# akamiru/bce

Measured on AMD Instinct MI355X. Metric: MB/s compressed, higher is better.
Workload: dtype u8/u32 integer

## Files before the change

bce_amd/csrc/common.h:

```cpp
#pragma once
#include <hip/hip_runtime.h>
#include <stdint.h>
#include <stdio.h>
#include <stdlib.h>
#include <string.h>

#include <atomic>
#include <chrono>
#include <condition_variable>
#include <exception>
#include <new>
#include <memory>
#include <mutex>
#include <thread>
#include <vector>

#include <sys/mman.h>

#include "../../include/bce_hip.h"
#include "bce_core.h"
#include "host_coder.h"

namespace bce {

// ... 194 lines not shown
    hipError_t _e = (expr);                                           \
    if (_e != hipSuccess) return bce::set_err((ctx), _e, #expr, __LINE__); \
  } while (0)

#define BCE_TRY(expr)                 \
  do {                                \
    int _rc = (expr);                 \
    if (_rc != BCE_HIP_OK) return _rc; \
  } while (0)

size_t ctx_trim(bce_hip_ctx *c);
inline bool test_oom_now() {
  static const char *e = getenv("BCE_HIP_TEST_OOM");
  static const unsigned long k = e ? strtoul(e, nullptr, 10) : 0;
  static std::atomic<unsigned long> count{0};
  return k && (count.fetch_add(1) + 1) % k == 0;
}
enum AllocSite { kAllocPlain = 0, kAllocListFirst = 1, kAllocListFallback = 2 };
inline bool test_oom_fails(const bce_hip_ctx *c, int site, int attempt) {
  switch (c->dbg_oom) {
    case 1: return site == kAllocListFirst;
    case 2: return site != kAllocPlain;
    case 3: return attempt == 0;
    default: return false;
  }
}
inline size_t test_oom_bytes(size_t bytes) {
  size_t fr = 0, tot = 0;
  if (hipMemGetInfo(&fr, &tot) != hipSuccess) { (void)hipGetLastError(); return bytes; }
  return tot + ((size_t)1 << 30);
}
inline int ensure(bce_hip_ctx *c, DevBuf &b, size_t bytes, int site = kAllocPlain) {
  if (bytes <= b.cap) return BCE_HIP_OK;
  if (b.p) {
    for (hipStream_t st : {c->stream, c->k4_stream, c->copy_stream}) if (st) BCE_HIP_TRY(c, hipStreamSynchronize(st));
    (void)hipFree(b.p);
    b.p = nullptr; b.cap = 0;
  }
  const double t0 = now_s();
  const bool hooked = c->dbg_oom != 0;
  hipError_t e = hipMalloc(&b.p, test_oom_fails(c, site, 0) ? test_oom_bytes(bytes) : bytes);
  const bool pretend = e == hipSuccess && test_oom_now();
  if (pretend) { (void)hipFree(b.p); e = hipErrorOutOfMemory; }
  if (e == hipErrorOutOfMemory) {
    (void)hipGetLastError();
    b.p = nullptr;
    if (ctx_trim(c) || pretend || hooked) e = hipMalloc(&b.p, test_oom_fails(c, site, 1) ? test_oom_bytes(bytes) : bytes);
  }
  if (e != hipSuccess) {
    b.p = nullptr;
    if (e == hipErrorOutOfMemory) (void)hipGetLastError();
    BCE_HIP_TRY(c, e);
  }
  c->alloc_s += now_s() - t0; c->alloc_bytes += bytes; c->alloc_calls++;
  if (now_s() - t0 > 0.02 && getenv("BCE_ALLOC_TRACE")) fprintf(stderr, "alloc: hipMalloc of %.1f MB took %.3f s\n", bytes / 1e6, now_s() - t0);
  b.cap = bytes;
  return BCE_HIP_OK;
}
inline int pin_alloc(bce_hip_ctx *c, void **p, size_t bytes) {
  const double t0 = now_s();
  BCE_HIP_TRY(c, hipHostMalloc(p, bytes, hipHostMallocDefault));
  c->pin_s += now_s() - t0; c->pin_bytes += bytes; c->pin_calls++;
  return BCE_HIP_OK;
}
inline void release(DevBuf &b) {
  if (b.p) (void)hipFree(b.p);
  b.p = nullptr; b.cap = 0;
}

inline int read_back(bce_hip_ctx *c, void *dst, const void *dev_src, size_t bytes) {
  if (bytes > 4096) return BCE_HIP_E_ARG;
  if (!c->h_small) BCE_TRY(pin_alloc(c, &c->h_small, 4096));
  BCE_HIP_TRY(c, hipMemcpyAsync(c->h_small, dev_src, bytes, hipMemcpyDeviceToHost, c->stream));
  BCE_HIP_TRY(c, hipStreamSynchronize(c->stream));
  memcpy(dst, c->h_small, bytes);
  return BCE_HIP_OK;
}

template <class F>
inline int bce_guarded(bce_hip_ctx *c, F &&body) {
  try { return body(); }
  catch (const std::bad_alloc &) { if (c) snprintf(c->err, sizeof c->err, "host allocation failed"); return BCE_HIP_E_NOMEM; }
  catch (const std::exception &e) { if (c) snprintf(c->err, sizeof c->err, "%s", e.what()); return BCE_HIP_E_INTERNAL; }
  catch (...) { if (c) snprintf(c->err, sizeof c->err, "unknown exception"); return BCE_HIP_E_INTERNAL; }
}

struct PhaseScope {
  PhaseScope(bce_hip_ctx *c, int phase) : c_(c) { c_->phase = phase; }
  ~PhaseScope() { c_->phase = 0; }
  PhaseScope(const PhaseScope &) = delete;
  PhaseScope &operator=(const PhaseScope &) = delete;
 private:
  bce_hip_ctx *c_;
};

struct RoctxRange {
  explicit RoctxRange(const char *name);
  ~RoctxRange();
  RoctxRange(const RoctxRange &) = delete;
  RoctxRange &operator=(const RoctxRange &) = delete;
 private:
  bool on_;
};

constexpr uint32_t K3_TAIL_CAP = 1024;
constexpr uint32_t K3_SMALL_MAXTILES = 2048;
#ifndef K3_SMALL_NODES_VALUE
#define K3_SMALL_NODES_VALUE 2000000u
#endif
constexpr uint32_t K3_SMALL_NODES = K3_SMALL_NODES_VALUE;
constexpr uint32_t K3_TAIL_ENTER = 512;
constexpr uint32_t K3_TAIL_MAXROUNDS = 65536;

inline uint32_t ceil_log2(uint32_t v) { uint32_t b = 0; while ((1ull << b) < v) ++b; return b; }

int k1_bwt(bce_hip_ctx *c);
int k1_divbwt(bce_hip_ctx *c, const uint8_t *T_host, uint8_t *U_host, uint32_t n, uint32_t *pidx);
int kd_inverse_bw_transform(bce_hip_ctx *c, const uint8_t *T_host, uint8_t *U_host, uint32_t n, uint32_t idx);
int kd_compare(bce_hip_ctx *c, const uint8_t *a, const uint8_t *b, uint64_t m, uint64_t *first_diff);
int kd_crc32(bce_hip_ctx *c, const uint8_t *d, uint64_t n, uint32_t *crc);
int k2_build_planes(bce_hip_ctx *c);
int k2_get_plane_bits(bce_hip_ctx *c, int plane, uint8_t *out);
int k2_rank1(bce_hip_ctx *c, int plane, const uint32_t *idx, uint32_t count, uint32_t *out);
int k3_begin(bce_hip_ctx *c);
int k3_rounds(bce_hip_ctx *c, uint32_t count, uint64_t nodes_hint);
int k3_rounds_small(bce_hip_ctx *c, uint32_t count, uint64_t cur_nodes, bool growing);
int k3_round_masked(bce_hip_ctx *c, uint32_t mask, bool repeat);
int k3_clear_need_flush(bce_hip_ctx *c);
int k3_clear_small_bail(bce_hip_ctx *c);
int k3_dfs_tail(bce_hip_ctx *c, const EnumCtl &ctl, uint32_t enter, bool *done);
int k3_tail(bce_hip_ctx *c, uint32_t max_rounds = K3_TAIL_MAXROUNDS);
int k3_fetch_tail_runs(bce_hip_ctx *c, uint32_t rounds);
int k3_sync_ctl(bce_hip_ctx *c, EnumCtl *out);
int k3_fetch_runs(bce_hip_ctx *c, uint32_t first_round, uint32_t count);
int k3_get_nodes(bce_hip_ctx *c, int plane, uint32_t *out, uint32_t cap, uint32_t *count);
int k3_reset_symbols(bce_hip_ctx *c);
int k3_grow_symbols(bce_hip_ctx *c, uint64_t cap);
int k4_prepare(bce_hip_ctx *c);
int k3_grow_lists(bce_hip_ctx *c, const EnumCtl &ctl);
uint64_t k3_symbol_capacity(const bce_hip_ctx *c, uint32_t n);
void k4_prepin(bce_hip_ctx *c, uint32_t n);
void k4_prepin_join(bce_hip_ctx *c, bool drop);
int k4_flush(bce_hip_ctx *c, uint64_t nsym, FlushSlot &slot);
int k4_flush_async(bce_hip_ctx *c, uint64_t nsym, FlushSlot &slot, bool copy_out = true);
int k4_long_runs(bce_hip_ctx *c, uint64_t nsym, uint32_t *count);
int k4_cost_begin(bce_hip_ctx *c);
int k4_cost_async(bce_hip_ctx *c, uint64_t nsym, FlushSlot &slot);
int k4_cost_end(bce_hip_ctx *c, uint64_t acc[16]);

int radix_sort_pairs(bce_hip_ctx *c, uint32_t *key[2], uint32_t *val[2], uint32_t n, uint32_t first_bit, uint32_t bits, int *res,
                     uint32_t max_digit_bits = 8);
int radix_sort_pairs_on(bce_hip_ctx *c, hipStream_t stream, DevBuf &hist, uint32_t *key[2], uint32_t *val[2], uint32_t n,
                        uint32_t first_bit, uint32_t bits, int *res, uint32_t max_digit_bits = 8);
int radix_sort_wide(bce_hip_ctx *c, uint32_t *lo[2], uint32_t *hi[2], uint32_t *val[2], uint32_t n, uint32_t bits, int *res,
                    uint32_t max_digit_bits = 10);
bool k4_in_flight(bce_hip_ctx *c);

}
```

bce_amd/csrc/k1_bwt.hip:

```cpp
#include <stdlib.h>

#include <utility>

#include "common.h"
#include "scan_util.h"

namespace bce {

#ifndef K1_ACT_TENTHS
#define K1_ACT_TENTHS 6
#endif

constexpr int K1_T = 256;

constexpr uint32_t K1_MAXB = 1024;
struct K1Plan { uint32_t nb, per_block; };
static K1Plan k1_plan(uint32_t n) {
  const uint32_t chunk = 2048;
  uint32_t chunks = (uint32_t)(((uint64_t)n + chunk - 1) / chunk);
  if (!chunks) chunks = 1;
  uint32_t nb = chunks < K1_MAXB ? chunks : K1_MAXB;
  uint32_t cpb = (chunks + nb - 1) / nb;
  nb = (chunks + cpb - 1) / cpb;
  return {nb, cpb * chunk};
// ... 569 lines not shown
  for (uint64_t i = (uint64_t)blockIdx.x * K1_T + threadIdx.x; i < m; i += (uint64_t)gridDim.x * K1_T)
    if (!(flag[i] & KF_DEFER)) rank[vs[i]] = nr[i];
}

template <int PASS, int MODE>
__global__ __launch_bounds__(K1_T) void k1_relist_kernel(const uint32_t *__restrict__ A, const uint32_t *__restrict__ vs,
                                                         const uint8_t *__restrict__ flag, uint32_t m,
                                                         uint32_t per_block, uint32_t nb, uint32_t *__restrict__ blockcnt,
                                                         uint32_t *__restrict__ out, uint32_t *__restrict__ out2, uint32_t *__restrict__ total,
                                                         uint32_t *__restrict__ blockcnt2 = nullptr, uint32_t *__restrict__ out3 = nullptr) {
  const uint64_t beg = (uint64_t)blockIdx.x * per_block;
  uint64_t end = beg + per_block;
  if (end > m) end = m;
  auto take = [&](uint64_t i) -> bool { return MODE == 0 ? (flag[i] & KF_DEFER) != 0 : (flag[i] & KF_KEEP) != 0; };
  if (PASS == 0) {
    uint32_t cnt = 0, hc = 0;
    for (uint64_t i = beg + threadIdx.x; i < end; i += K1_T) {
      const bool k = take(i);
      cnt += k ? 1u : 0u;
      if (MODE == 0) hc += (k && (A[i] & K1_HEAD)) ? 1u : 0u;
    }
    cnt = block_reduce_sum<K1_T>(cnt);
    if (MODE == 0) hc = block_reduce_sum<K1_T>(hc);
    if (threadIdx.x == 0) { blockcnt[blockIdx.x] = cnt; if (MODE == 0) blockcnt2[blockIdx.x] = hc; }
  } else {
    uint32_t b = 0, a = 0, b2 = 0, a2 = 0;
    for (uint32_t k = threadIdx.x; k < nb; k += K1_T) {
      const uint32_t v = blockcnt[k];
      a += v; if (k < blockIdx.x) b += v;
      if (MODE == 0) { const uint32_t v2 = blockcnt2[k]; a2 += v2; if (k < blockIdx.x) b2 += v2; }
    }
    uint32_t base = block_reduce_sum<K1_T>(b);
    const uint32_t all = block_reduce_sum<K1_T>(a);
    uint32_t hbase = 0;
    if (MODE == 0) {
      hbase = block_reduce_sum<K1_T>(b2);
      const uint32_t all2 = block_reduce_sum<K1_T>(a2);
      if (blockIdx.x == 0 && threadIdx.x == 0) total[1] = all2;
    }
    if (blockIdx.x == 0 && threadIdx.x == 0) total[0] = all;
    for (uint64_t c0 = beg; c0 < end; c0 += K1_T) {
      const uint64_t i = c0 + threadIdx.x;
      const bool k = i < end && take(i);
      const uint32_t a_i = (MODE == 0 && k) ? A[i] : 0u;
      uint32_t tot;
      const uint32_t ex = block_excl_scan_sum<K1_T>(k ? 1u : 0u, &tot);
      uint32_t htot = 0, hex = 0;
      const uint32_t hd = (MODE == 0 && (a_i & K1_HEAD)) ? 1u : 0u;
      if (MODE == 0) hex = block_excl_scan_sum<K1_T>(hd, &htot);
      if (k) {
        if (MODE == 0) { out[base + ex] = (uint32_t)i; out2[base + ex] = a_i & K1_SLOT; out3[base + ex] = hbase + hex + hd - 1u; }
        else { out[base + ex] = (A[i] & K1_SLOT) | ((flag[i] & KF_HEAD) ? K1_HEAD : 0u); out2[base + ex] = vs[i]; }
      }
      base += tot;
      hbase += htot;
    }
  }
}

__global__ __launch_bounds__(K1_T) void k1_big_gather_kernel(const uint32_t *__restrict__ idx, const uint32_t *__restrict__ gid,
                                                             const uint32_t *__restrict__ V, const uint32_t *__restrict__ rank,
                                                             uint32_t n, uint32_t nd, uint32_t h, uint32_t rbits,
                                                             uint32_t *__restrict__ lo, uint32_t *__restrict__ hi, uint32_t *__restrict__ val) {
  for (uint64_t j = (uint64_t)blockIdx.x * K1_T + threadIdx.x; j < nd; j += (uint64_t)gridDim.x * K1_T) {
    const uint32_t p = V[idx[j]];
    uint64_t q = (uint64_t)p + h;
    if (q >= n) q -= n;
    const uint64_t key = ((uint64_t)gid[j] << rbits) | rank[q];
    lo[j] = (uint32_t)key;
    hi[j] = (uint32_t)(key >> 32);
    val[j] = p;
  }
}
__global__ __launch_bounds__(K1_T) void k1_big_heads_kernel(const uint32_t *__restrict__ slots, const uint32_t *__restrict__ lo,
                                                            const uint32_t *__restrict__ hi, const uint32_t *__restrict__ val,
                                                            uint32_t nd, uint32_t per_block, uint32_t *__restrict__ sa,
                                                            uint32_t *__restrict__ nrk, uint32_t *__restrict__ blockmax) {
  const uint64_t beg = (uint64_t)blockIdx.x * per_block;
  uint64_t end = beg + per_block;
  if (end > nd) end = nd;
  uint32_t mx = 0;
  for (uint64_t j = beg + threadIdx.x; j < end; j += K1_T) {
    const uint32_t slot = slots[j];
    sa[slot] = val[j];
    const bool head = j == 0 || lo[j] != lo[j - 1] || hi[j] != hi[j - 1];
    nrk[j] = head ? slot : 0u;
    if (head) mx = slot;
  }
  mx = block_reduce_max<K1_T>(mx);
  if (threadIdx.x == 0) blockmax[blockIdx.x] = mx;
}

__global__ __launch_bounds__(K1_T) void k1_defer_flags_kernel(const uint32_t *__restrict__ nrk, const uint32_t *__restrict__ idx,
                                                              const uint32_t *__restrict__ sorted, uint32_t nd,
                                                              uint8_t *__restrict__ flag, uint32_t *__restrict__ vs) {
  for (uint64_t j = (uint64_t)blockIdx.x * K1_T + threadIdx.x; j < nd; j += (uint64_t)gridDim.x * K1_T) {
    const bool hd = j == 0 || nrk[j] != 0u;
    const bool nx = j + 1 >= nd || nrk[j + 1] != 0u;
    const uint32_t i = idx[j];
    flag[i] = (uint8_t)(KF_DEFER | (hd ? KF_HEAD : 0) | ((hd && nx) ? 0 : KF_KEEP));
    vs[i] = sorted[j];
  }
}

static int k1_sort_rotations(bce_hip_ctx *c, const uint8_t *T, uint32_t n, bool sentinel) {
  if (getenv("BCE_K1_V1")) return k1_sort_rotations_v1(c, T, n, sentinel);
  const size_t b4 = (size_t)n * 4;
  for (int i = 0; i < 2; ++i) { BCE_TRY(ensure(c, c->sa[i], b4)); BCE_TRY(ensure(c, c->key[i], b4)); BCE_TRY(ensure(c, c->khi[i], b4)); }
  BCE_TRY(ensure(c, c->rank, b4));
  BCE_TRY(ensure(c, c->k2, b4));
  BCE_TRY(ensure(c, c->nrk, b4));
  BCE_TRY(ensure(c, c->kflag, (size_t)n + 16));
  for (int i = 0; i < 2; ++i) { BCE_TRY(ensure(c, c->act[i], b4)); BCE_TRY(ensure(c, c->actv[i], b4)); }
  const K1Plan pl = k1_plan(n);
  BCE_TRY(ensure(c, c->blk, (size_t)(K1_MAXB + K1_SC_CODE + 128 + K1_MAXB) * 4));
  uint32_t *blockmax = c->blk.as<uint32_t>();
  uint32_t *scalars = blockmax + K1_MAXB;
  uint32_t *rank = c->rank.as<uint32_t>(), *k2 = c->k2.as<uint32_t>(), *nrk = c->nrk.as<uint32_t>();
  uint8_t *flag = c->kflag.as<uint8_t>();
  const uint32_t g = grid_for(n);
  const bool trace = getenv("BCE_K1_TRACE") != nullptr;
  double t_prev = now_s();
  auto lap = [&](const char *what, uint64_t h, uint32_t m, uint32_t nd) {
    if (!trace) return;
    (void)hipStreamSynchronize(c->stream);
    const double t = now_s();
    fprintf(stderr, "k1 %p: %-10s h %llu active %u deferred %u (+%.2f ms)\n", (void *)c, what, (unsigned long long)h, m, nd, (t - t_prev) * 1e3);
    t_prev = t;
  };

  const uint32_t nbytes = sentinel ? n - 1u : n;
  BCE_HIP_TRY(c, hipMemsetAsync(scalars + K1_SC_HIST, 0, 256 * 4, c->stream));
  hipLaunchKernelGGL(k1_bytehist_kernel, dim3(g < 1024u ? g : 1024u), dim3(K1_T), 0, c->stream, T, nbytes, scalars + K1_SC_HIST);
  uint32_t hist[256];
  BCE_TRY(read_back(c, hist, scalars + K1_SC_HIST, sizeof hist));
  uint16_t code[256];
  uint32_t sigma = sentinel ? 1u : 0u;
  for (int b = 0; b < 256; ++b) { code[b] = (uint16_t)sigma; if (hist[b]) ++sigma; }
  uint32_t bits = ceil_log2(sigma);
  if (bits < 1) bits = 1;
  uint32_t nsym = 64u / bits;
  if (nsym > 16u) nsym = 16u;
  if (const char *e = getenv("BCE_K1_KEYBITS")) { const uint32_t v = (uint32_t)strtoul(e, nullptr, 10); if (v >= bits && v / bits < nsym) nsym = v / bits; }
  const uint32_t keybits = nsym * bits;
  {
    if (!c->h_small) BCE_TRY(pin_alloc(c, &c->h_small, 4096));
    memcpy(c->h_small, code, sizeof code);
    BCE_HIP_TRY(c, hipMemcpyAsync(scalars + K1_SC_CODE, c->h_small, sizeof code, hipMemcpyHostToDevice, c->stream));
  }

  uint32_t *lo[2] = {c->key[0].as<uint32_t>(), c->key[1].as<uint32_t>()};
  uint32_t *hi[2] = {c->khi[0].as<uint32_t>(), c->khi[1].as<uint32_t>()};
  uint32_t *val[2] = {c->sa[0].as<uint32_t>(), c->sa[1].as<uint32_t>()};
  {
    const uint32_t per = K1_T * K1I_E;
    hipLaunchKernelGGL(k1_init64_kernel, dim3((uint32_t)(((uint64_t)n + per - 1) / per)), dim3(K1_T), 0, c->stream, T, n, nbytes,
                       reinterpret_cast<const uint16_t *>(scalars + K1_SC_CODE), bits, nsym, lo[0], hi[0], val[0]);
  }
  int res = 0;
  BCE_TRY(radix_sort_wide(c, lo, hi, val, n, keybits, &res, 9));
  lap("first sort", nsym, n, 0);
  BCE_HIP_TRY(c, hipMemsetAsync(scalars, 0, 16, c->stream));
  hipLaunchKernelGGL(k1_heads_kernel, dim3(pl.nb), dim3(K1_T), 0, c->stream, hi[res], lo[res], n, pl.per_block, nrk, blockmax, scalars);
  const uint32_t rbits = ceil_log2(n);
  static const uint32_t part_min = getenv("BCE_K1_PART_MIN") ? (uint32_t)strtoul(getenv("BCE_K1_PART_MIN"), nullptr, 10) : K1_PART_MIN;
  const bool sorted_apply = n >= part_min;
  if (sorted_apply) hipLaunchKernelGGL(k1_headidx_kernel, dim3(pl.nb), dim3(K1_T), 0, c->stream, nrk, blockmax, n, pl.per_block, k2);
  else hipLaunchKernelGGL(k1_apply_kernel, dim3(pl.nb), dim3(K1_T), 0, c->stream, nrk, blockmax, n, pl.per_block, val[res], rank);
  uint32_t *act[2] = {c->act[0].as<uint32_t>(), c->act[1].as<uint32_t>()};
  uint32_t *actv[2] = {c->actv[0].as<uint32_t>(), c->actv[1].as<uint32_t>()};
  uint32_t m = 0;
  hipLaunchKernelGGL(k1_active_kernel<0>, dim3(pl.nb), dim3(K1_T), 0, c->stream, nrk, (const uint32_t *)nullptr, n, pl.per_block, pl.nb,
                     blockmax, act[0], scalars + 2, 1u, (const uint32_t *)val[res], actv[0]);
  hipLaunchKernelGGL(k1_active_kernel<1>, dim3(pl.nb), dim3(K1_T), 0, c->stream, nrk, (const uint32_t *)nullptr, n, pl.per_block, pl.nb,
                     blockmax, act[0], scalars + 2, 1u, (const uint32_t *)val[res], actv[0]);
  if (sorted_apply) {
    const uint32_t b1 = rbits / ((rbits + 9u) / 10u);
    uint32_t *pk[2] = {val[res], lo[res ^ 1]}, *pv[2] = {k2, rank};
    int pr = 0;
    BCE_TRY(radix_sort_pairs(c, pk, pv, n, 0, b1, &pr, 10));
    uint32_t *qk[2] = {lo[res ^ 1], hi[res ^ 1]}, *qv[2] = {rank, val[res ^ 1]};
    BCE_TRY(radix_sort_pairs(c, qk, qv, n, b1, rbits - b1, &pr, 10));
    if (pr) BCE_HIP_TRY(c, hipMemcpyAsync(rank, qv[1], (size_t)n * 4, hipMemcpyDeviceToDevice, c->stream));
  }
  BCE_TRY(read_back(c, &m, scalars + 2, 4));
  lap("first ranks", nsym, m, 0);

  uint64_t h = nsym;
  uint32_t *sa = val[res];
  uint32_t *nr = hi[0], *vs = hi[1];
  while (m > 0 && h < n) {
    const uint32_t *A = act[0];
    const uint32_t nblk = (uint32_t)(((uint64_t)m + SEG_CH - 1) / SEG_CH);
    BCE_HIP_TRY(c, hipMemsetAsync(scalars + 3, 0, 4, c->stream));
    hipLaunchKernelGGL(k1_seg_sort_kernel, dim3(nblk), dim3(SEG_T), 0, c->stream, A, (const uint32_t *)actv[0], m, sa, rank, n, (uint32_t)h, nr, vs,
                       flag, scalars + 3);
    uint32_t nd = 0;
    BCE_TRY(read_back(c, &nd, scalars + 3, 4));
    const K1Plan ap = k1_plan(m);
    if (nd) {
      BCE_TRY(ensure(c, c->dl[0], (size_t)nd * 4));
      BCE_TRY(ensure(c, c->dl[1], (size_t)nd * 4));
      BCE_TRY(ensure(c, c->dl[2], (size_t)nd * 4));
      BCE_TRY(ensure(c, c->dl[3], (size_t)nd * 4));
      uint32_t *idx = c->dl[0].as<uint32_t>(), *slots = c->dl[1].as<uint32_t>(), *gid = c->dl[2].as<uint32_t>();
      uint32_t *blockcnt2 = scalars + K1_SC_CODE + 128;
      hipLaunchKernelGGL((k1_relist_kernel<0, 0>), dim3(ap.nb), dim3(K1_T), 0, c->stream, A, (const uint32_t *)vs, flag, m, ap.per_block, ap.nb, blockmax, idx, slots,
                         scalars + 4, blockcnt2, gid);
      hipLaunchKernelGGL((k1_relist_kernel<1, 0>), dim3(ap.nb), dim3(K1_T), 0, c->stream, A, (const uint32_t *)vs, flag, m, ap.per_block, ap.nb, blockmax, idx, slots,
                         scalars + 4, blockcnt2, gid);
      uint32_t cnts[2] = {0, 0};
      BCE_TRY(read_back(c, cnts, scalars + 4, 8));
      if (cnts[0] != nd || cnts[1] == 0 || cnts[1] > nd) { snprintf(c->err, sizeof c->err, "k1: deferred list %u / %u groups, expected %u elements", cnts[0], cnts[1], nd); return BCE_HIP_E_INTERNAL; }
      const uint32_t gbits = ceil_log2(cnts[1]);
      uint32_t *bl[2] = {lo[0], lo[1]};
      uint32_t *bh[2] = {val[res ^ 1], k2};
      uint32_t *bv[2] = {nrk, c->dl[3].as<uint32_t>()};
      const uint32_t ga = grid_for(nd);
      hipLaunchKernelGGL(k1_big_gather_kernel, dim3(ga), dim3(K1_T), 0, c->stream, idx, gid, (const uint32_t *)actv[0], rank, n, nd, (uint32_t)h, rbits,
                         bl[0], bh[0], bv[0]);
      int rb = 0;
      BCE_TRY(radix_sort_wide(c, bl, bh, bv, nd, rbits + gbits, &rb, 9));
      const K1Plan dp = k1_plan(nd);
      uint32_t *snrk = bv[rb ^ 1];
      hipLaunchKernelGGL(k1_big_heads_kernel, dim3(dp.nb), dim3(K1_T), 0, c->stream, slots, bl[rb], bh[rb], bv[rb], nd, dp.per_block, sa, snrk, blockmax);
      hipLaunchKernelGGL(k1_act_apply_kernel, dim3(dp.nb), dim3(K1_T), 0, c->stream, snrk, blockmax, nd, dp.per_block, bv[rb], rank);
      uint32_t *vjr = bv[rb];
      hipLaunchKernelGGL(k1_defer_flags_kernel, dim3(ga), dim3(K1_T), 0, c->stream, snrk, idx, (const uint32_t *)vjr, nd, flag, vs);
    }
    if (m >= part_min) {
      const uint32_t b1 = rbits / ((rbits + 9u) / 10u);
      uint32_t *pk[2] = {lo[0], lo[1]}, *pv[2] = {nr, k2};
      hipLaunchKernelGGL(k1_seg_pairs_kernel, dim3(grid_for(m)), dim3(K1_T), 0, c->stream, (const uint32_t *)vs, (const uint8_t *)flag, KF_DEFER, m, pk[0]);
      int pr = 0;
      BCE_TRY(radix_sort_pairs(c, pk, pv, m, 0, b1, &pr, 10));
      uint32_t *qk[2] = {lo[1], lo[0]}, *qv[2] = {k2, val[res ^ 1]};
      BCE_TRY(radix_sort_pairs(c, qk, qv, m, b1, rbits - b1, &pr, 10));
      hipLaunchKernelGGL(k1_scatter32_kernel, dim3(grid_for(m)), dim3(K1_T), 0, c->stream, (const uint32_t *)qk[pr], (const uint32_t *)qv[pr], m, n, rank);
    } else {
      hipLaunchKernelGGL(k1_seg_apply_kernel, dim3(grid_for(m)), dim3(K1_T), 0, c->stream, nr, vs, flag, m, rank);
    }
    hipLaunchKernelGGL((k1_relist_kernel<0, 1>), dim3(ap.nb), dim3(K1_T), 0, c->stream, A, (const uint32_t *)vs, flag, m, ap.per_block, ap.nb, blockmax, act[1],
                       actv[1], scalars + 2);
    hipLaunchKernelGGL((k1_relist_kernel<1, 1>), dim3(ap.nb), dim3(K1_T), 0, c->stream, A, (const uint32_t *)vs, flag, m, ap.per_block, ap.nb, blockmax, act[1],
                       actv[1], scalars + 2);
    const uint32_t m_old = m;
    BCE_TRY(read_back(c, &m, scalars + 2, 4));
    std::swap(act[0], act[1]);
    std::swap(actv[0], actv[1]);
    h <<= 1;
    c->stats.sort_rounds++;
    lap("round", h, m, nd);
    (void)m_old;
  }
  BCE_HIP_TRY(c, hipGetLastError());
  c->k1_unique = m == 0;
  c->sa_res = res;
  return BCE_HIP_OK;
}

int k1_bwt(bce_hip_ctx *c) {
  const uint32_t n = c->n;
  uint8_t *T = c->text.as<uint8_t>();
  BCE_TRY(ensure(c, c->bwt, n));
  uint8_t *bwt = c->bwt.as<uint8_t>();
  c->stats.sort_rounds = 0;
  c->k1_unique = false;
  c->k1_valid = false;
  if (n == 1) {
    BCE_HIP_TRY(c, hipMemcpyAsync(bwt, T, 1, hipMemcpyDeviceToDevice, c->stream));
    BCE_HIP_TRY(c, hipStreamSynchronize(c->stream));
    c->offset = 0;
    return BCE_HIP_OK;
  }
  BCE_TRY(k1_sort_rotations(c, T, n, false));
  const uint32_t g = grid_for(n);
  uint32_t *scalars = c->blk.as<uint32_t>() + K1_MAXB;
  const uint32_t *sa = c->sa[c->sa_res].as<uint32_t>();
  BCE_HIP_TRY(c, hipMemsetAsync(scalars + 1, 0xFF, 4, c->stream));
  hipLaunchKernelGGL(k1_bwt_kernel, dim3(g), dim3(K1_T), 0, c->stream, T, sa, n, bwt);
  hipLaunchKernelGGL(k1_offset_kernel, dim3(g), dim3(K1_T), 0, c->stream, c->rank.as<uint32_t>(), n, scalars + 1);
  uint32_t off = 0;
  BCE_TRY(read_back(c, &off, scalars + 1, 4));
  BCE_HIP_TRY(c, hipGetLastError());
  if (off >= n) { snprintf(c->err, sizeof c->err, "k1: no rank-0 rotation found"); return BCE_HIP_E_INTERNAL; }
  c->offset = off;
  c->k1_valid = true;
  return BCE_HIP_OK;
}

__global__ __launch_bounds__(K1_T) void k1_divbwt_gather_kernel(const uint8_t *__restrict__ T, const uint32_t *__restrict__ sa,
                                                                uint32_t m, uint32_t pidx, uint8_t *__restrict__ U) {
  for (uint64_t j = (uint64_t)blockIdx.x * K1_T + threadIdx.x; j < m; j += (uint64_t)gridDim.x * K1_T) {
    const uint32_t p = sa[j];
    if (p != 0u) U[j < pidx ? j : j - 1u] = T[p - 1u];
  }
}

int k1_divbwt(bce_hip_ctx *c, const uint8_t *T_host, uint8_t *U_host, uint32_t n, uint32_t *pidx_out) {
  if (n == 0 || n >= 0x7FFFFFFFu) return BCE_HIP_E_ARG;
  const uint32_t m = n + 1u;
  c->stage = 0; c->k1_valid = false; c->enum_active = false; c->text_loaded = false;
  BCE_TRY(ensure(c, c->text, m));
  BCE_TRY(ensure(c, c->bwt, m));
  uint8_t *T = c->text.as<uint8_t>();
  BCE_HIP_TRY(c, hipMemcpyAsync(T, T_host, n, hipMemcpyHostToDevice, c->stream));
  c->stats.sort_rounds = 0;
  BCE_TRY(k1_sort_rotations(c, T, m, true));
  uint32_t pidx = 0;
  BCE_TRY(read_back(c, &pidx, c->rank.as<uint32_t>(), 4));
  if (pidx == 0 || pidx > n) { snprintf(c->err, sizeof c->err, "divbwt: primary index %u out of range", pidx); return BCE_HIP_E_INTERNAL; }
  hipLaunchKernelGGL(k1_divbwt_gather_kernel, dim3(grid_for(m)), dim3(K1_T), 0, c->stream, T, c->sa[c->sa_res].as<uint32_t>(), m,
                     pidx, c->bwt.as<uint8_t>());
// ... 9 lines not shown
```

bce_amd/csrc/radix_sort.hip:

```cpp
#include "common.h"
#include "scan_util.h"

namespace bce {

constexpr int RS_THREADS = 256;
constexpr int RS_ITEMS = 16;
constexpr int RS_CHUNK = RS_THREADS * RS_ITEMS;
constexpr int RS_MAXB = 768;
constexpr int RS_MAXBITS = 10;
constexpr int RS_MAXBINS = 1 << RS_MAXBITS;

struct RsPlan { uint32_t nb, per_block; };
static RsPlan rs_plan(uint32_t n) {
  uint32_t chunks = (uint32_t)(((uint64_t)n + RS_CHUNK - 1) / RS_CHUNK);
  if (chunks == 0) chunks = 1;
  uint32_t nb = chunks < (uint32_t)RS_MAXB ? chunks : (uint32_t)RS_MAXB;
  uint32_t cpb = (chunks + nb - 1) / nb;
  nb = (chunks + cpb - 1) / cpb;
  return {nb, cpb * (uint32_t)RS_CHUNK};
}

template <int NBITS>
__device__ __forceinline__ uint64_t match_digit(uint32_t d, int nbits, bool valid) {
  const uint64_t vm = __ballot(valid);
// ... 54 lines not shown
        atomicAdd(&lh[w][d], 1u);
      }
    }
  }
  __syncthreads();
  for (uint32_t d = tid; d < nbins; d += RS_THREADS) hist[(size_t)d * nb + blockIdx.x] = lh[0][d] + lh[1][d] + lh[2][d] + lh[3][d];
}

__global__ __launch_bounds__(RS_THREADS) void rs_scan_kernel(uint32_t *__restrict__ hist, uint32_t nb,
                                                             uint32_t *__restrict__ rowtotal) {
  uint32_t *row = hist + (size_t)blockIdx.x * nb;
  uint32_t carry = 0;
  for (uint32_t base = 0; base < nb; base += RS_THREADS) {
    const uint32_t i = base + threadIdx.x;
    const uint32_t v = i < nb ? row[i] : 0u;
    uint32_t tot;
    const uint32_t ex = block_excl_scan_sum<RS_THREADS>(v, &tot);
    if (i < nb) row[i] = carry + ex;
    carry += tot;
  }
  if (threadIdx.x == 0) rowtotal[blockIdx.x] = carry;
}

template <int NBITS>
__global__ __launch_bounds__(RS_THREADS) void rs_scatter_kernel(const uint32_t *__restrict__ keys_in,
                                                                const uint32_t *__restrict__ vals_in,
                                                                uint32_t *__restrict__ keys_out,
                                                                uint32_t *__restrict__ vals_out, uint32_t n,
                                                                uint32_t per_block, uint32_t nb, int shift, int nbits,
                                                                const uint32_t *__restrict__ hist,
                                                                const uint32_t *__restrict__ rowtotal) {
  constexpr int BINS = NBITS > 0 ? (1 << NBITS) : RS_MAXBINS;
  __shared__ uint32_t wcnt[4][BINS];
  __shared__ uint32_t goff[BINS];
  __shared__ uint32_t gdelta[BINS];
  __shared__ uint32_t skey[RS_CHUNK], sval[RS_CHUNK];
  constexpr int BPT = (BINS + RS_THREADS - 1) / RS_THREADS;
  const uint32_t tid = threadIdx.x, lane = tid & 63u, w = tid >> 6;
  const uint32_t nbins = 1u << nbits, mask = nbins - 1u;
  {
    uint32_t v[BPT], sum = 0;
#pragma unroll
    for (int q = 0; q < BPT; ++q) {
      const uint32_t d = tid * BPT + q;
      v[q] = d < nbins ? rowtotal[d] : 0u;
      sum += v[q];
    }
    uint32_t tot;
    uint32_t run = block_excl_scan_sum<RS_THREADS>(sum, &tot);
#pragma unroll
    for (int q = 0; q < BPT; ++q) {
      const uint32_t d = tid * BPT + q;
      if (d < nbins) goff[d] = run + hist[(size_t)d * nb + blockIdx.x];
      run += v[q];
    }
  }
  const uint64_t beg = (uint64_t)blockIdx.x * per_block;
  uint64_t end = beg + per_block;
  if (end > n) end = n;
  const uint64_t lt = (1ull << lane) - 1ull;
  for (uint64_t base = beg; base < end; base += RS_CHUNK) {
    const uint32_t cnt = (uint32_t)(end - base < (uint64_t)RS_CHUNK ? end - base : (uint64_t)RS_CHUNK);
    for (uint32_t d = tid; d < nbins; d += RS_THREADS) { wcnt[0][d] = 0; wcnt[1][d] = 0; wcnt[2][d] = 0; wcnt[3][d] = 0; }
    __syncthreads();
    uint32_t key[RS_ITEMS], val[RS_ITEMS], lr[RS_ITEMS];
#pragma unroll
    for (int it = 0; it < RS_ITEMS; ++it) {
      const uint32_t q = w * (RS_CHUNK / 4) + (uint32_t)it * 64u + lane;
      const bool valid = q < cnt;
      key[it] = valid ? keys_in[base + q] : 0u;
      val[it] = valid ? vals_in[base + q] : 0u;
    }
#pragma unroll
    for (int it = 0; it < RS_ITEMS; ++it) {
      const uint32_t q = w * (RS_CHUNK / 4) + (uint32_t)it * 64u + lane;
      const bool valid = q < cnt;
      const uint32_t d = (key[it] >> shift) & mask;
      const uint64_t peers = match_digit<NBITS>(d, nbits, valid);
      const uint32_t leader = valid ? (uint32_t)(__ffsll((long long)peers) - 1) : lane;
      uint32_t pre = 0;
      if (valid && lane == leader) pre = atomicAdd(&wcnt[w][d], (uint32_t)__popcll(peers));
      pre = __shfl(pre, (int)leader);
      lr[it] = pre + (uint32_t)__popcll(peers & lt);
    }
    __syncthreads();
    {
      uint32_t c[BPT][4], sum = 0;
#pragma unroll
      for (int q = 0; q < BPT; ++q) {
        const uint32_t d = tid * BPT + q;
#pragma unroll
        for (int ww = 0; ww < 4; ++ww) { c[q][ww] = d < nbins ? wcnt[ww][d] : 0u; sum += c[q][ww]; }
      }
      uint32_t tot;
      uint32_t run = block_excl_scan_sum<RS_THREADS>(sum, &tot);
#pragma unroll
      for (int q = 0; q < BPT; ++q) {
        const uint32_t d = tid * BPT + q;
        if (d < nbins) {
          const uint32_t t4 = c[q][0] + c[q][1] + c[q][2] + c[q][3];
          wcnt[0][d] = run; wcnt[1][d] = run + c[q][0]; wcnt[2][d] = run + c[q][0] + c[q][1];
          wcnt[3][d] = run + c[q][0] + c[q][1] + c[q][2];
          const uint32_t g = goff[d];
          gdelta[d] = g - run;
          goff[d] = g + t4;
          run += t4;
        }
      }
    }
    __syncthreads();
#pragma unroll
    for (int it = 0; it < RS_ITEMS; ++it) {
      const uint32_t q = w * (RS_CHUNK / 4) + (uint32_t)it * 64u + lane;
      if (q < cnt) {
        const uint32_t d = (key[it] >> shift) & mask;
        const uint32_t pos = wcnt[w][d] + lr[it];
        skey[pos] = key[it];
        sval[pos] = val[it];
      }
    }
    __syncthreads();
#pragma unroll
    for (int it = 0; it < RS_ITEMS; ++it) {
      const uint32_t q = (uint32_t)it * RS_THREADS + tid;
      if (q < cnt) {
        const uint32_t k = skey[q];
        const uint32_t pos = gdelta[(k >> shift) & mask] + q;
        keys_out[pos] = k;
        vals_out[pos] = sval[q];
      }
    }
    __syncthreads();
  }
}

#ifndef RW_ITEMS_VALUE
#define RW_ITEMS_VALUE 8
#endif
constexpr int RW_ITEMS = RW_ITEMS_VALUE;
constexpr int RW_CHUNK = RS_THREADS * RW_ITEMS;
static RsPlan rw_plan(uint32_t n) {
  uint32_t chunks = (uint32_t)(((uint64_t)n + RW_CHUNK - 1) / RW_CHUNK);
  if (chunks == 0) chunks = 1;
  const uint32_t maxb = RW_ITEMS <= 8 ? 1024 : 768;
  uint32_t nb = chunks < maxb ? chunks : maxb;
  uint32_t cpb = (chunks + nb - 1) / nb;
  nb = (chunks + cpb - 1) / cpb;
  return {nb, cpb * (uint32_t)RW_CHUNK};
}
__device__ __forceinline__ uint32_t digit64(uint32_t lo, uint32_t hi, int shift, uint32_t mask) {
  return (uint32_t)((((uint64_t)hi << 32) | lo) >> shift) & mask;
}

__global__ __launch_bounds__(RS_THREADS) void rw_hist_kernel(const uint32_t *__restrict__ lo, const uint32_t *__restrict__ hi,
                                                             uint32_t n, uint32_t per_block, uint32_t nb, int shift, int nbits,
                                                             uint32_t *__restrict__ hist) {
  __shared__ uint32_t lh[4][RS_MAXBINS];
  const uint32_t tid = threadIdx.x, lane = tid & 63u, w = tid >> 6;
  const uint32_t nbins = 1u << nbits, mask = nbins - 1u;
  for (uint32_t d = tid; d < nbins; d += RS_THREADS) { lh[0][d] = 0; lh[1][d] = 0; lh[2][d] = 0; lh[3][d] = 0; }
  __syncthreads();
  const uint64_t beg = (uint64_t)blockIdx.x * per_block;
  uint64_t end = beg + per_block;
  if (end > n) end = n;
  const bool need_lo = shift < 32, need_hi = shift + nbits > 32;
  for (uint64_t base = beg; base < end; base += (uint64_t)RS_THREADS * 16) {
    uint32_t kl[16], kh[16];
#pragma unroll
    for (int it = 0; it < 16; ++it) {
      const uint64_t i = base + (uint64_t)it * RS_THREADS + tid;
      kl[it] = (need_lo && i < end) ? lo[i] : 0u;
      kh[it] = (need_hi && i < end) ? hi[i] : 0u;
    }
#pragma unroll
    for (int it = 0; it < 16; ++it) {
      const uint64_t i = base + (uint64_t)it * RS_THREADS + tid;
      const bool valid = i < end;
      const uint32_t d = digit64(kl[it], kh[it], shift, mask);
      const uint32_t d0 = (uint32_t)__builtin_amdgcn_readfirstlane((int)d);
      if (__all(valid && d == d0)) {
        if (lane == 0) atomicAdd(&lh[w][d0], 64u);
      } else if (valid) {
        atomicAdd(&lh[w][d], 1u);
      }
    }
  }
  __syncthreads();
  for (uint32_t d = tid; d < nbins; d += RS_THREADS) hist[(size_t)d * nb + blockIdx.x] = lh[0][d] + lh[1][d] + lh[2][d] + lh[3][d];
}

template <int NBITS>
__global__ __launch_bounds__(RS_THREADS) void rw_scatter_kernel(const uint32_t *__restrict__ lo_in, const uint32_t *__restrict__ hi_in,
                                                                const uint32_t *__restrict__ vals_in,
                                                                uint32_t *__restrict__ lo_out, uint32_t *__restrict__ hi_out,
                                                                uint32_t *__restrict__ vals_out, uint32_t n,
                                                                uint32_t per_block, uint32_t nb, int shift, int nbits,
                                                                const uint32_t *__restrict__ hist,
                                                                const uint32_t *__restrict__ rowtotal) {
  constexpr int BINS = NBITS > 0 ? (1 << NBITS) : RS_MAXBINS;
  __shared__ uint32_t wcnt[4][BINS];
  __shared__ uint32_t goff[BINS];
  __shared__ uint32_t gdelta[BINS];
  __shared__ uint32_t slo[RW_CHUNK], shi[RW_CHUNK], sval[RW_CHUNK];
  constexpr int BPT = (BINS + RS_THREADS - 1) / RS_THREADS;
  const uint32_t tid = threadIdx.x, lane = tid & 63u, w = tid >> 6;
  const uint32_t nbins = 1u << nbits, mask = nbins - 1u;
  {
    uint32_t v[BPT], sum = 0;
#pragma unroll
    for (int q = 0; q < BPT; ++q) {
      const uint32_t d = tid * BPT + q;
      v[q] = d < nbins ? rowtotal[d] : 0u;
      sum += v[q];
    }
    uint32_t tot;
    uint32_t run = block_excl_scan_sum<RS_THREADS>(sum, &tot);
#pragma unroll
    for (int q = 0; q < BPT; ++q) {
      const uint32_t d = tid * BPT + q;
      if (d < nbins) goff[d] = run + hist[(size_t)d * nb + blockIdx.x];
      run += v[q];
    }
  }
  const uint64_t beg = (uint64_t)blockIdx.x * per_block;
  uint64_t end = beg + per_block;
  if (end > n) end = n;
  const uint64_t lt = (1ull << lane) - 1ull;
  for (uint64_t base = beg; base < end; base += RW_CHUNK) {
    const uint32_t cnt = (uint32_t)(end - base < (uint64_t)RW_CHUNK ? end - base : (uint64_t)RW_CHUNK);
    for (uint32_t d = tid; d < nbins; d += RS_THREADS) { wcnt[0][d] = 0; wcnt[1][d] = 0; wcnt[2][d] = 0; wcnt[3][d] = 0; }
    __syncthreads();
    uint32_t kl[RW_ITEMS], kh[RW_ITEMS], val[RW_ITEMS], lr[RW_ITEMS];
#pragma unroll
    for (int it = 0; it < RW_ITEMS; ++it) {
      const uint32_t q = w * (RW_CHUNK / 4) + (uint32_t)it * 64u + lane;
      const bool valid = q < cnt;
      kl[it] = valid ? lo_in[base + q] : 0u;
      kh[it] = valid ? hi_in[base + q] : 0u;
      val[it] = valid ? vals_in[base + q] : 0u;
    }
#pragma unroll
    for (int it = 0; it < RW_ITEMS; ++it) {
      const uint32_t q = w * (RW_CHUNK / 4) + (uint32_t)it * 64u + lane;
      const bool valid = q < cnt;
      const uint32_t d = digit64(kl[it], kh[it], shift, mask);
      const uint64_t peers = match_digit<NBITS>(d, nbits, valid);
      const uint32_t leader = valid ? (uint32_t)(__ffsll((long long)peers) - 1) : lane;
      uint32_t pre = 0;
      if (valid && lane == leader) pre = atomicAdd(&wcnt[w][d], (uint32_t)__popcll(peers));
      pre = __shfl(pre, (int)leader);
      lr[it] = pre + (uint32_t)__popcll(peers & lt);
    }
    __syncthreads();
    {
      uint32_t c[BPT][4], sum = 0;
#pragma unroll
      for (int q = 0; q < BPT; ++q) {
        const uint32_t d = tid * BPT + q;
#pragma unroll
        for (int ww = 0; ww < 4; ++ww) { c[q][ww] = d < nbins ? wcnt[ww][d] : 0u; sum += c[q][ww]; }
      }
      uint32_t tot;
      uint32_t run = block_excl_scan_sum<RS_THREADS>(sum, &tot);
#pragma unroll
      for (int q = 0; q < BPT; ++q) {
        const uint32_t d = tid * BPT + q;
        if (d < nbins) {
          const uint32_t t4 = c[q][0] + c[q][1] + c[q][2] + c[q][3];
          wcnt[0][d] = run; wcnt[1][d] = run + c[q][0]; wcnt[2][d] = run + c[q][0] + c[q][1];
          wcnt[3][d] = run + c[q][0] + c[q][1] + c[q][2];
          const uint32_t g = goff[d];
          gdelta[d] = g - run;
          goff[d] = g + t4;
          run += t4;
        }
      }
    }
    __syncthreads();
#pragma unroll
    for (int it = 0; it < RW_ITEMS; ++it) {
      const uint32_t q = w * (RW_CHUNK / 4) + (uint32_t)it * 64u + lane;
      if (q < cnt) {
        const uint32_t d = digit64(kl[it], kh[it], shift, mask);
        const uint32_t pos = wcnt[w][d] + lr[it];
        slo[pos] = kl[it];
        shi[pos] = kh[it];
        sval[pos] = val[it];
      }
    }
    __syncthreads();
#pragma unroll
    for (int it = 0; it < RW_ITEMS; ++it) {
      const uint32_t q = (uint32_t)it * RS_THREADS + tid;
      if (q < cnt) {
        const uint32_t l = slo[q], hh = shi[q];
        const uint32_t pos = gdelta[digit64(l, hh, shift, mask)] + q;
        lo_out[pos] = l;
        hi_out[pos] = hh;
        vals_out[pos] = sval[q];
      }
    }
    __syncthreads();
  }
}

int radix_sort_wide(bce_hip_ctx *c, uint32_t *lo[2], uint32_t *hi[2], uint32_t *val[2], uint32_t n, uint32_t bits, int *res,
                    uint32_t max_digit_bits) {
  *res = 0;
  if (n <= 1 || bits == 0) return BCE_HIP_OK;
  if (bits > 64) return BCE_HIP_E_ARG;
  if (max_digit_bits < 1 || max_digit_bits > (uint32_t)RS_MAXBITS) max_digit_bits = 8;
  const RsPlan pl = rw_plan(n);
  BCE_TRY(ensure(c, c->rs_hist, ((size_t)RS_MAXBINS * pl.nb + RS_MAXBINS) * sizeof(uint32_t)));
  uint32_t *hist = c->rs_hist.as<uint32_t>();
  uint32_t *rowtotal = hist + (size_t)RS_MAXBINS * pl.nb;
  const uint32_t npass = (bits + max_digit_bits - 1) / max_digit_bits;
  int cur = 0;
  uint32_t done = 0;
  for (uint32_t pass = 0; pass < npass; ++pass) {
    const uint32_t left = bits - done, pleft = npass - pass;
    const int nbits = (int)((left + pleft - 1) / pleft);
    const uint32_t nbins = 1u << nbits;
    hipLaunchKernelGGL(rw_hist_kernel, dim3(pl.nb), dim3(RS_THREADS), 0, c->stream, lo[cur], hi[cur], n, pl.per_block, pl.nb,
                       (int)done, nbits, hist);
    hipLaunchKernelGGL(rs_scan_kernel, dim3(nbins), dim3(RS_THREADS), 0, c->stream, hist, pl.nb, rowtotal);
#define RW_SCATTER(NB)                                                                                                      \
  hipLaunchKernelGGL(rw_scatter_kernel<NB>, dim3(pl.nb), dim3(RS_THREADS), 0, c->stream, lo[cur], hi[cur], val[cur], lo[cur ^ 1], \
                     hi[cur ^ 1], val[cur ^ 1], n, pl.per_block, pl.nb, (int)done, nbits, hist, rowtotal)
    switch (nbits) {
      case 10: RW_SCATTER(10); break;
      case 9: RW_SCATTER(9); break;
      case 8: RW_SCATTER(8); break;
      case 7: RW_SCATTER(7); break;
      default: RW_SCATTER(0); break;
    }
#undef RW_SCATTER
    cur ^= 1;
    done += (uint32_t)nbits;
  }
  BCE_HIP_TRY(c, hipGetLastError());
  *res = cur;
  return BCE_HIP_OK;
}

int radix_sort_pairs(bce_hip_ctx *c, uint32_t *key[2], uint32_t *val[2], uint32_t n, uint32_t first_bit, uint32_t bits,
                     int *res, uint32_t max_digit_bits) {
  return radix_sort_pairs_on(c, c->stream, c->rs_hist, key, val, n, first_bit, bits, res, max_digit_bits);
}

int radix_sort_pairs_on(bce_hip_ctx *c, hipStream_t stream, DevBuf &hbuf, uint32_t *key[2], uint32_t *val[2], uint32_t n,
                        uint32_t first_bit, uint32_t bits, int *res, uint32_t max_digit_bits) {
  *res = 0;
  if ((uint64_t)first_bit + bits > 32) {
    snprintf(c->err, sizeof c->err, "radix sort: key bits [%u, %u + %u) do not lie inside 32", first_bit, first_bit, bits);
    return BCE_HIP_E_ARG;
  }
  if (n <= 1 || bits == 0) return BCE_HIP_OK;
  if (max_digit_bits < 1 || max_digit_bits > (uint32_t)RS_MAXBITS) max_digit_bits = 8;
  const RsPlan pl = rs_plan(n);
  BCE_TRY(ensure(c, hbuf, ((size_t)RS_MAXBINS * pl.nb + RS_MAXBINS) * sizeof(uint32_t)));
  uint32_t *hist = hbuf.as<uint32_t>();
  uint32_t *rowtotal = hist + (size_t)RS_MAXBINS * pl.nb;
  const uint32_t npass = (bits + max_digit_bits - 1) / max_digit_bits;
  int cur = 0;
  uint32_t done = 0;
  for (uint32_t pass = 0; pass < npass; ++pass) {
    const uint32_t left = bits - done, pleft = npass - pass;
    const int nbits = (int)((left + pleft - 1) / pleft);
    const uint32_t shift = first_bit + done;
    const uint32_t nbins = 1u << nbits;
    hipLaunchKernelGGL(rs_hist_kernel, dim3(pl.nb), dim3(RS_THREADS), 0, stream, key[cur], n, pl.per_block, pl.nb,
                       (int)shift, nbits, hist);
    hipLaunchKernelGGL(rs_scan_kernel, dim3(nbins), dim3(RS_THREADS), 0, stream, hist, pl.nb, rowtotal);
#define RS_SCATTER(NB)                                                                                              \
  hipLaunchKernelGGL(rs_scatter_kernel<NB>, dim3(pl.nb), dim3(RS_THREADS), 0, stream, key[cur], val[cur], key[cur ^ 1], \
                     val[cur ^ 1], n, pl.per_block, pl.nb, (int)shift, nbits, hist, rowtotal)
    switch (nbits) {
      case 10: RS_SCATTER(10); break;
      case 9: RS_SCATTER(9); break;
      case 8: RS_SCATTER(8); break;
      case 7: RS_SCATTER(7); break;
      case 6: RS_SCATTER(6); break;
      default: RS_SCATTER(0); break;
    }
#undef RS_SCATTER
    cur ^= 1;
    done += (uint32_t)nbits;
  }
  BCE_HIP_TRY(c, hipGetLastError());
  *res = cur;
  return BCE_HIP_OK;
}

}
```

Before: 855.3.

## Fuse k1 key construction into first radix pass reading text directly

Drops the separate init64 kernel that materialized 64-bit packed symbol keys and suffix indices. Instead, the first histogram and scatter passes of the wide radix sort build keys on the fly from the input text through a shared-memory code lookup table. This saves one full write and read of the lo/hi/val arrays. In exchange, the histogram recomputes its low digits from text bytes and the scatter builds a symbol window in shared memory, which adds some compute and reuses the slo buffer.

```diff
diff --git a/bce_amd/csrc/common.h b/bce_amd/csrc/common.h
--- a/bce_amd/csrc/common.h
+++ b/bce_amd/csrc/common.h
@@ -370,8 +370,14 @@
                      uint32_t max_digit_bits = 8);
 int radix_sort_pairs_on(bce_hip_ctx *c, hipStream_t stream, DevBuf &hist, uint32_t *key[2], uint32_t *val[2], uint32_t n,
                         uint32_t first_bit, uint32_t bits, int *res, uint32_t max_digit_bits = 8);
+struct RwText {
+  const uint8_t *T;
+  const uint16_t *code;
+  uint32_t nbytes;
+  uint32_t bits, nsym;
+};
 int radix_sort_wide(bce_hip_ctx *c, uint32_t *lo[2], uint32_t *hi[2], uint32_t *val[2], uint32_t n, uint32_t bits, int *res,
-                    uint32_t max_digit_bits = 10);
+                    uint32_t max_digit_bits = 10, const RwText *text = nullptr);
 bool k4_in_flight(bce_hip_ctx *c);
 
 }
diff --git a/bce_amd/csrc/k1_bwt.hip b/bce_amd/csrc/k1_bwt.hip
--- a/bce_amd/csrc/k1_bwt.hip
+++ b/bce_amd/csrc/k1_bwt.hip
@@ -745,13 +745,18 @@
   uint32_t *lo[2] = {c->key[0].as<uint32_t>(), c->key[1].as<uint32_t>()};
   uint32_t *hi[2] = {c->khi[0].as<uint32_t>(), c->khi[1].as<uint32_t>()};
   uint32_t *val[2] = {c->sa[0].as<uint32_t>(), c->sa[1].as<uint32_t>()};
-  {
+  const char *dknob = getenv("BCE_K1_DIRECT");
+  const bool direct = n > 1 && !(dknob && dknob[0] == '0' && dknob[1] == 0);
+  if (trace) fprintf(stderr, "k1 %p: path %s n %u sigma %u bits %u nsym %u\n", (void *)c, direct ? "direct" : "init64", n, sigma, bits, nsym);
+  const uint16_t *dcode = reinterpret_cast<const uint16_t *>(scalars + K1_SC_CODE);
+  const RwText tx = {T, dcode, nbytes, bits, nsym};
+  if (!direct) {
     const uint32_t per = K1_T * K1I_E;
     hipLaunchKernelGGL(k1_init64_kernel, dim3((uint32_t)(((uint64_t)n + per - 1) / per)), dim3(K1_T), 0, c->stream, T, n, nbytes,
-                       reinterpret_cast<const uint16_t *>(scalars + K1_SC_CODE), bits, nsym, lo[0], hi[0], val[0]);
+                       dcode, bits, nsym, lo[0], hi[0], val[0]);
   }
   int res = 0;
-  BCE_TRY(radix_sort_wide(c, lo, hi, val, n, keybits, &res, 9));
+  BCE_TRY(radix_sort_wide(c, lo, hi, val, n, keybits, &res, 9, direct ? &tx : nullptr));
   lap("first sort", nsym, n, 0);
   BCE_HIP_TRY(c, hipMemsetAsync(scalars, 0, 16, c->stream));
   hipLaunchKernelGGL(k1_heads_kernel, dim3(pl.nb), dim3(K1_T), 0, c->stream, hi[res], lo[res], n, pl.per_block, nrk, blockmax, scalars);
diff --git a/bce_amd/csrc/radix_sort.hip b/bce_amd/csrc/radix_sort.hip
--- a/bce_amd/csrc/radix_sort.hip
+++ b/bce_amd/csrc/radix_sort.hip
@@ -230,13 +230,18 @@
   return (uint32_t)((((uint64_t)hi << 32) | lo) >> shift) & mask;
 }
 
+__device__ __forceinline__ uint64_t rw_wrap(uint64_t q, uint32_t m) { return q >= m ? q % m : q; }
+
+template <bool TEXT>
 __global__ __launch_bounds__(RS_THREADS) void rw_hist_kernel(const uint32_t *__restrict__ lo, const uint32_t *__restrict__ hi,
                                                              uint32_t n, uint32_t per_block, uint32_t nb, int shift, int nbits,
-                                                             uint32_t *__restrict__ hist) {
+                                                             uint32_t *__restrict__ hist, RwText tx) {
   __shared__ uint32_t lh[4][RS_MAXBINS];
+  __shared__ uint16_t lut[TEXT ? 256 : 1];
   const uint32_t tid = threadIdx.x, lane = tid & 63u, w = tid >> 6;
   const uint32_t nbins = 1u << nbits, mask = nbins - 1u;
   for (uint32_t d = tid; d < nbins; d += RS_THREADS) { lh[0][d] = 0; lh[1][d] = 0; lh[2][d] = 0; lh[3][d] = 0; }
+  if (TEXT) lut[tid] = tx.code[tid];
   __syncthreads();
   const uint64_t beg = (uint64_t)blockIdx.x * per_block;
   uint64_t end = beg + per_block;
@@ -244,11 +249,28 @@
   const bool need_lo = shift < 32, need_hi = shift + nbits > 32;
   for (uint64_t base = beg; base < end; base += (uint64_t)RS_THREADS * 16) {
     uint32_t kl[16], kh[16];
-#pragma unroll
-    for (int it = 0; it < 16; ++it) {
-      const uint64_t i = base + (uint64_t)it * RS_THREADS + tid;
-      kl[it] = (need_lo && i < end) ? lo[i] : 0u;
-      kh[it] = (need_hi && i < end) ? hi[i] : 0u;
+    if (TEXT) {
+      const uint32_t nlow = ((uint32_t)nbits + tx.bits - 1u) / tx.bits;
+#pragma unroll
+      for (int it = 0; it < 16; ++it) { kl[it] = 0u; kh[it] = 0u; }
+      for (uint32_t b = tx.nsym - nlow; b < tx.nsym; ++b) {
+        uint32_t by[16];
+#pragma unroll
+        for (int it = 0; it < 16; ++it) {
+          const uint64_t i = base + (uint64_t)it * RS_THREADS + tid;
+          const uint64_t q = rw_wrap(i + b, n);
+          by[it] = (i < end && q < tx.nbytes) ? (uint32_t)tx.T[q] : 256u;
+        }
+#pragma unroll
+        for (int it = 0; it < 16; ++it) kl[it] = (kl[it] << tx.bits) | (by[it] < 256u ? (uint32_t)lut[by[it]] : 0u);
+      }
+    } else {
+#pragma unroll
+      for (int it = 0; it < 16; ++it) {
+        const uint64_t i = base + (uint64_t)it * RS_THREADS + tid;
+        kl[it] = (need_lo && i < end) ? lo[i] : 0u;
+        kh[it] = (need_hi && i < end) ? hi[i] : 0u;
+      }
     }
 #pragma unroll
     for (int it = 0; it < 16; ++it) {
@@ -267,19 +289,24 @@
   for (uint32_t d = tid; d < nbins; d += RS_THREADS) hist[(size_t)d * nb + blockIdx.x] = lh[0][d] + lh[1][d] + lh[2][d] + lh[3][d];
 }
 
-template <int NBITS>
+constexpr int RW_SYM_PAD = 16;
+static_assert((RW_CHUNK + RW_SYM_PAD) * 2 <= RW_CHUNK * 4, "the symbol window must fit the low-word stage");
+template <int NBITS, bool TEXT>
 __global__ __launch_bounds__(RS_THREADS) void rw_scatter_kernel(const uint32_t *__restrict__ lo_in, const uint32_t *__restrict__ hi_in,
                                                                 const uint32_t *__restrict__ vals_in,
                                                                 uint32_t *__restrict__ lo_out, uint32_t *__restrict__ hi_out,
                                                                 uint32_t *__restrict__ vals_out, uint32_t n,
                                                                 uint32_t per_block, uint32_t nb, int shift, int nbits,
                                                                 const uint32_t *__restrict__ hist,
-                                                                const uint32_t *__restrict__ rowtotal) {
+                                                                const uint32_t *__restrict__ rowtotal, RwText tx) {
   constexpr int BINS = NBITS > 0 ? (1 << NBITS) : RS_MAXBINS;
   __shared__ uint32_t wcnt[4][BINS];
   __shared__ uint32_t goff[BINS];
   __shared__ uint32_t gdelta[BINS];
-  __shared__ uint32_t slo[RW_CHUNK], shi[RW_CHUNK], sval[RW_CHUNK];
+  __shared__ __attribute__((aligned(16))) uint32_t slo[RW_CHUNK];
+  __shared__ uint32_t shi[RW_CHUNK], sval[RW_CHUNK];
+  __shared__ uint16_t lut[TEXT ? 256 : 1];
+  if (TEXT) lut[threadIdx.x] = tx.code[threadIdx.x];
   constexpr int BPT = (BINS + RS_THREADS - 1) / RS_THREADS;
   const uint32_t tid = threadIdx.x, lane = tid & 63u, w = tid >> 6;
   const uint32_t nbins = 1u << nbits, mask = nbins - 1u;
@@ -309,13 +336,49 @@
     for (uint32_t d = tid; d < nbins; d += RS_THREADS) { wcnt[0][d] = 0; wcnt[1][d] = 0; wcnt[2][d] = 0; wcnt[3][d] = 0; }
     __syncthreads();
     uint32_t kl[RW_ITEMS], kh[RW_ITEMS], val[RW_ITEMS], lr[RW_ITEMS];
-#pragma unroll
-    for (int it = 0; it < RW_ITEMS; ++it) {
-      const uint32_t q = w * (RW_CHUNK / 4) + (uint32_t)it * 64u + lane;
-      const bool valid = q < cnt;
-      kl[it] = valid ? lo_in[base + q] : 0u;
-      kh[it] = valid ? hi_in[base + q] : 0u;
-      val[it] = valid ? vals_in[base + q] : 0u;
+    if (TEXT) {
+      uint16_t *sym = reinterpret_cast<uint16_t *>(slo);
+      const uint32_t need = cnt + tx.nsym - 1u;
+      if (base + RW_CHUNK + RW_SYM_PAD <= (uint64_t)tx.nbytes && (reinterpret_cast<uintptr_t>(tx.T) & 3u) == 0) {
+        const uint32_t *T4 = reinterpret_cast<const uint32_t *>(tx.T + base);
+        uint32_t *sym2 = slo;
+        for (uint32_t i = tid; i < (RW_CHUNK + RW_SYM_PAD) / 4; i += RS_THREADS) {
+          const uint32_t v = T4[i];
+          sym2[2 * i] = (uint32_t)lut[v & 255u] | ((uint32_t)lut[(v >> 8) & 255u] << 16);
+          sym2[2 * i + 1] = (uint32_t)lut[(v >> 16) & 255u] | ((uint32_t)lut[v >> 24] << 16);
+        }
+      } else {
+        for (uint32_t i = tid; i < need; i += RS_THREADS) {
+          const uint64_t q = rw_wrap(base + i, n);
+          sym[i] = q < tx.nbytes ? lut[tx.T[q]] : (uint16_t)0;
+        }
+      }
+      __syncthreads();
+      uint64_t k[RW_ITEMS];
+#pragma unroll
+      for (int it = 0; it < RW_ITEMS; ++it) k[it] = 0;
+      for (uint32_t b = 0; b < tx.nsym; ++b) {
+#pragma unroll
+        for (int it = 0; it < RW_ITEMS; ++it)
+          k[it] = (k[it] << tx.bits) | sym[w * (RW_CHUNK / 4) + (uint32_t)it * 64u + lane + b];
+      }
+#pragma unroll
+      for (int it = 0; it < RW_ITEMS; ++it) {
+        const uint32_t q = w * (RW_CHUNK / 4) + (uint32_t)it * 64u + lane;
+        const bool valid = q < cnt;
+        kl[it] = valid ? (uint32_t)k[it] : 0u;
+        kh[it] = valid ? (uint32_t)(k[it] >> 32) : 0u;
+        val[it] = valid ? (uint32_t)(base + q) : 0u;
+      }
+    } else {
+#pragma unroll
+      for (int it = 0; it < RW_ITEMS; ++it) {
+        const uint32_t q = w * (RW_CHUNK / 4) + (uint32_t)it * 64u + lane;
+        const bool valid = q < cnt;
+        kl[it] = valid ? lo_in[base + q] : 0u;
+        kh[it] = valid ? hi_in[base + q] : 0u;
+        val[it] = valid ? vals_in[base + q] : 0u;
+      }
     }
 #pragma unroll
     for (int it = 0; it < RW_ITEMS; ++it) {
@@ -383,8 +446,11 @@
 }
 
 int radix_sort_wide(bce_hip_ctx *c, uint32_t *lo[2], uint32_t *hi[2], uint32_t *val[2], uint32_t n, uint32_t bits, int *res,
-                    uint32_t max_digit_bits) {
+                    uint32_t max_digit_bits, const RwText *text) {
   *res = 0;
+  if (text && (n <= 1 || bits == 0 || text->bits == 0 || text->bits > 16 || text->nsym == 0 || text->nsym > (uint32_t)RW_SYM_PAD ||
+               text->bits * text->nsym != bits || text->nbytes > n || n - text->nbytes > 1))
+    return BCE_HIP_E_ARG;
   if (n <= 1 || bits == 0) return BCE_HIP_OK;
   if (bits > 64) return BCE_HIP_E_ARG;
   if (max_digit_bits < 1 || max_digit_bits > (uint32_t)RS_MAXBITS) max_digit_bits = 8;
@@ -399,12 +465,19 @@
     const uint32_t left = bits - done, pleft = npass - pass;
     const int nbits = (int)((left + pleft - 1) / pleft);
     const uint32_t nbins = 1u << nbits;
-    hipLaunchKernelGGL(rw_hist_kernel, dim3(pl.nb), dim3(RS_THREADS), 0, c->stream, lo[cur], hi[cur], n, pl.per_block, pl.nb,
-                       (int)done, nbits, hist);
+    const bool from_text = text && pass == 0;
+    const RwText tx = from_text ? *text : RwText{};
+    if (from_text)
+      hipLaunchKernelGGL(rw_hist_kernel<true>, dim3(pl.nb), dim3(RS_THREADS), 0, c->stream, lo[cur], hi[cur], n, pl.per_block, pl.nb,
+                         (int)done, nbits, hist, tx);
+    else
+      hipLaunchKernelGGL(rw_hist_kernel<false>, dim3(pl.nb), dim3(RS_THREADS), 0, c->stream, lo[cur], hi[cur], n, pl.per_block, pl.nb,
+                         (int)done, nbits, hist, tx);
     hipLaunchKernelGGL(rs_scan_kernel, dim3(nbins), dim3(RS_THREADS), 0, c->stream, hist, pl.nb, rowtotal);
-#define RW_SCATTER(NB)                                                                                                      \
-  hipLaunchKernelGGL(rw_scatter_kernel<NB>, dim3(pl.nb), dim3(RS_THREADS), 0, c->stream, lo[cur], hi[cur], val[cur], lo[cur ^ 1], \
-                     hi[cur ^ 1], val[cur ^ 1], n, pl.per_block, pl.nb, (int)done, nbits, hist, rowtotal)
+#define RW_SCATTER_AS(NB, TX)                                                                                               \
+  hipLaunchKernelGGL((rw_scatter_kernel<NB, TX>), dim3(pl.nb), dim3(RS_THREADS), 0, c->stream, lo[cur], hi[cur], val[cur], lo[cur ^ 1], \
+                     hi[cur ^ 1], val[cur ^ 1], n, pl.per_block, pl.nb, (int)done, nbits, hist, rowtotal, tx)
+#define RW_SCATTER(NB) do { if (from_text) RW_SCATTER_AS(NB, true); else RW_SCATTER_AS(NB, false); } while (0)
     switch (nbits) {
       case 10: RW_SCATTER(10); break;
       case 9: RW_SCATTER(9); break;
@@ -413,6 +486,7 @@
       default: RW_SCATTER(0); break;
     }
 #undef RW_SCATTER
+#undef RW_SCATTER_AS
     cur ^= 1;
     done += (uint32_t)nbits;
   }
```

Result: no change. 853.4 (-0.2%).
